# IlzeAmandaA/VAE-GP-ODE

Hardware: NVIDIA B200
Metric: GP-ODE RK4 latent traj-steps/s fwd+bwd (higher is better)
Workload: dtype f32

## Files before the change

### vae-gp-ode_b200/csrc/rbf_bwd_tc.cuh

```cuda
#pragma once

#include <cuda_bf16.h>
#include <cuda_fp16.h>

#include "rbf_kernels.cuh"
#include "tc_common.cuh"

namespace gpode {

#ifndef GPODE_BT_SLEEP_NS
#define GPODE_BT_SLEEP_NS 64
#endif
#ifndef GPODE_BT_A_TMEM
#define GPODE_BT_A_TMEM 1
#endif
constexpr int kBtACol = 448;
#ifndef GPODE_BT_EXP
#define GPODE_BT_EXP 0
#endif

constexpr int kBtStates = 128;
constexpr int kBtEpiWarps = 16;
constexpr int kBtEpi = kBtEpiWarps * 32;
constexpr int kBtFlushWarps = 4;
constexpr int kBtThreads = kBtEpi + 64 + 32 * kBtFlushWarps + 64;
constexpr int kBtPgIssuer = kBtEpiWarps + 2 + kBtFlushWarps;
constexpr int kBtThIssuer = kBtPgIssuer + 1;
constexpr int kBtTauBytes = 2 * 16 * 2048;
constexpr int kBtABytes = 3 * 4096;
constexpr int kBtXpBytes = 6 * 2048;
constexpr int kBtQCol = 256, kBtPgCol = 352;
constexpr int kBtNBars = 26;
constexpr uint32_t kBtOffTau = 0, kBtOffTh = 2 * kBtTauBytes, kBtOffP = kBtOffTh + 2 * kTcbThBytes, kBtOffA = kBtOffP + 2 * kTcbPBytes, kBtOffXp = kBtOffA + kBtABytes,
                   kBtOffXs = kBtOffXp + kBtXpBytes;

__host__ __device__ constexpr uint32_t tc_idesc_f16(int M, int N) {
  return (1u << 4) | (static_cast<uint32_t>(N >> 3) << 17) | (static_cast<uint32_t>(M >> 4) << 24);
}
__host__ __device__ constexpr uint32_t tc_idesc_bf16(int M, int N, int a_mn, int b_mn) {
  return (1u << 4) | (1u << 7) | (1u << 10) | (static_cast<uint32_t>(a_mn) << 15) | (static_cast<uint32_t>(b_mn) << 16) | (static_cast<uint32_t>(N >> 3) << 17) |
         (static_cast<uint32_t>(M >> 4) << 24);
}
__device__ __forceinline__ uint64_t tc_desc2(uint32_t saddr, uint32_t lbo_bytes, uint32_t sbo_bytes) {
  return static_cast<uint64_t>((saddr & 0x3FFFF) >> 4) | (static_cast<uint64_t>((lbo_bytes >> 4) & 0x3FFF) << 16) | (static_cast<uint64_t>((sbo_bytes >> 4) & 0x3FFF) << 32) |
         (static_cast<uint64_t>(1) << 46);
}
__device__ __forceinline__ void tcu_mma_f16(uint32_t d, uint64_t a, uint64_t b, uint32_t idesc, uint32_t acc) {
  asm volatile("{\n.reg .pred p, e;\nsetp.ne.b32 p, %4, 0;\nelect.sync _|e, 0xffffffff;\n@e tcgen05.mma.cta_group::1.kind::f16 [%0], %1, %2, %3, p;\n}\n" ::"r"(d), "l"(a), "l"(b),
               "r"(idesc), "r"(acc)
               : "memory");
}
__device__ __forceinline__ void tcu_mma_tf32(uint32_t d, uint64_t a, uint64_t b, uint32_t idesc, uint32_t acc) {
  asm volatile("{\n.reg .pred p, e;\nsetp.ne.b32 p, %4, 0;\nelect.sync _|e, 0xffffffff;\n@e tcgen05.mma.cta_group::1.kind::tf32 [%0], %1, %2, %3, p;\n}\n" ::"r"(d), "l"(a), "l"(b),
               "r"(idesc), "r"(acc)
               : "memory");
}
__device__ __forceinline__ void tcu_mma_f16_ts(uint32_t d, uint32_t a_tmem, uint64_t b, uint32_t idesc, uint32_t acc) {
  asm volatile("{\n.reg .pred p, e;\nsetp.ne.b32 p, %4, 0;\nelect.sync _|e, 0xffffffff;\n@e tcgen05.mma.cta_group::1.kind::f16 [%0], [%1], %2, %3, p;\n}\n" ::"r"(d), "r"(a_tmem),
               "l"(b), "r"(idesc), "r"(acc)
               : "memory");
}
__device__ __forceinline__ void tcu_mma_tf32_ts(uint32_t d, uint32_t a_tmem, uint64_t b, uint32_t idesc, uint32_t acc) {
  asm volatile("{\n.reg .pred p, e;\nsetp.ne.b32 p, %4, 0;\nelect.sync _|e, 0xffffffff;\n@e tcgen05.mma.cta_group::1.kind::tf32 [%0], [%1], %2, %3, p;\n}\n" ::"r"(d), "r"(a_tmem),
               "l"(b), "r"(idesc), "r"(acc)
               : "memory");
}
__device__ __forceinline__ void tc_st8(uint32_t taddr, const uint32_t (&r)[8]) {
  asm volatile("tcgen05.st.sync.aligned.32x32b.x8.b32 [%0], {%1,%2,%3,%4,%5,%6,%7,%8};" ::"r"(taddr), "r"(r[0]), "r"(r[1]), "r"(r[2]), "r"(r[3]), "r"(r[4]), "r"(r[5]),
               "r"(r[6]), "r"(r[7])
               : "memory");
}
__device__ __forceinline__ void tcu_commit(uint32_t bar) {
  asm volatile("{\n.reg .pred e;\nelect.sync _|e, 0xffffffff;\n@e tcgen05.commit.cta_group::1.mbarrier::arrive::one.shared::cluster.b64 [%0];\n}\n" ::"r"(bar) : "memory");
}
__device__ __forceinline__ void tc_ld4(uint32_t taddr, float (&v)[4]) {
  uint32_t r0, r1, r2, r3;
  asm volatile("tcgen05.ld.sync.aligned.32x32b.x4.b32 {%0,%1,%2,%3}, [%4];" : "=r"(r0), "=r"(r1), "=r"(r2), "=r"(r3) : "r"(taddr));
  asm volatile("tcgen05.wait::ld.sync.aligned;" : "+r"(r0), "+r"(r1), "+r"(r2), "+r"(r3)::"memory");
  v[0] = __uint_as_float(r0);
  v[1] = __uint_as_float(r1);
  v[2] = __uint_as_float(r2);
  v[3] = __uint_as_float(r3);
}
__device__ __forceinline__ void tc_ld2(uint32_t taddr, float (&v)[2]) {
  uint32_t r0, r1;
  asm volatile("tcgen05.ld.sync.aligned.32x32b.x2.b32 {%0,%1}, [%2];" : "=r"(r0), "=r"(r1) : "r"(taddr));
  asm volatile("tcgen05.wait::ld.sync.aligned;" : "+r"(r0), "+r"(r1)::"memory");
  v[0] = __uint_as_float(r0);
  v[1] = __uint_as_float(r1);
}
__device__ __forceinline__ void tc_ld4_async(uint32_t taddr, uint32_t& r0, uint32_t& r1, uint32_t& r2, uint32_t& r3) {
  asm volatile("tcgen05.ld.sync.aligned.32x32b.x4.b32 {%0,%1,%2,%3}, [%4];" : "=r"(r0), "=r"(r1), "=r"(r2), "=r"(r3) : "r"(taddr));
}
__device__ __forceinline__ void tc_ld2_async(uint32_t taddr, uint32_t& r0, uint32_t& r1) {
  asm volatile("tcgen05.ld.sync.aligned.32x32b.x2.b32 {%0,%1}, [%2];" : "=r"(r0), "=r"(r1) : "r"(taddr));
}
__device__ __forceinline__ void tc_ld_fence(uint32_t (&r)[10]) {
  asm volatile("" : "+r"(r[0]), "+r"(r[1]), "+r"(r[2]), "+r"(r[3]), "+r"(r[4]), "+r"(r[5]), "+r"(r[6]), "+r"(r[7]), "+r"(r[8]), "+r"(r[9])::"memory");
}
__device__ __forceinline__ void sts128(uint32_t saddr, uint32_t a, uint32_t b, uint32_t c, uint32_t d) {
#if GPODE_BT_EXP
  if (GPODE_BT_EXP & 8) {
    asm volatile("" ::"r"(saddr), "r"(a), "r"(b), "r"(c), "r"(d));
    return;
  }
#endif
  asm volatile("st.shared.v4.b32 [%0], {%1,%2,%3,%4};" ::"r"(saddr), "r"(a), "r"(b), "r"(c), "r"(d) : "memory");
}
__device__ __forceinline__ void bt_split2(float v0, float v1, uint32_t& hd, uint32_t& rm) {
  hd = __byte_perm(__float_as_uint(v0), __float_as_uint(v1), 0x7632);
  const float2 l = fma2(make_float2(__uint_as_float(__float_as_uint(v0) & 0xFFFF0000u), __uint_as_float(__float_as_uint(v1) & 0xFFFF0000u)), bc(-1.f), make_float2(v0, v1));
  asm("cvt.rn.bf16x2.f32 %0, %1, %2;" : "=r"(rm) : "f"(l.y), "f"(l.x));
}

#ifdef GPODE_BT_PROFILE
#define BT_E0 long long et_[12] = {0, 0, 0, 0, 0, 0, 0, 0, 0, 0, 0, 0}, ec_ = clock64();
#define BT_E(i) { const long long now_ = clock64(); et_[i] += now_ - ec_; ec_ = now_; }
#define BT_EPRINT if (blockIdx.x == 5 && blockIdx.y == 0 && b0 == static_cast<long>(n) && (tid == 0 || tid == 480)) \
  printf("bwd tc epilogue warp %d (cycles per item): first wait %lld, wait tau_empty %lld, ld issue + ld wait + arrives %lld, math+store %lld (+ wait next theta %lld), k setup + xprime %lld (+ wait xp_empty %lld), pg red %lld (+ waits pg_full / q_full %lld), q epilogue %lld (+ %lld)\n", warp, \
         et_[0] / n, et_[1] / n, et_[2] / n, et_[3] / n, et_[7] / n, et_[4] / n, et_[8] / n, et_[5] / n, et_[9] / n, et_[6] / n, et_[10] / n);
#define BT_I0 long long it_[8] = {0, 0, 0, 0, 0, 0, 0, 0}, ic_ = clock64();
#define BT_I(i) { const long long now_ = clock64(); it_[i] += now_ - ic_; ic_ = now_; }
#define BT_IPRINT if (blockIdx.x == 5 && blockIdx.y == 0 && b0 == static_cast<long>(n) && lane == 0) \
  printf("bwd tc issuer (cycles per item): theta waits (tile, acc_empty) %lld, theta issue %lld, wait tau_full %lld, wait p tile %lld, wait q_empty/xp/pg_empty %lld, issue Q %lld, issue PG %lld\n", \
         it_[0] / n, it_[1] / n, it_[2] / n, it_[3] / n, it_[4] / n, it_[5] / n, it_[6] / n);
#else
#define BT_E0
#define BT_E(i)
#define BT_EPRINT
#define BT_I0
#define BT_I(i)
#define BT_IPRINT
#endif

struct BwdTcSmem {
  unsigned char* tau;
  unsigned char* th;
  unsigned char* pp;
  unsigned char* A;
  unsigned char* xp;
  float* xs;
  float* dx;
  float* hdr;
  float* dell;
  float* dvar;
  float* sk;
  float* gs;
  float* g_pg;
  float* g_dnu;
  uint64_t* bars;
  uint32_t sb;
  uint32_t sbars;
  uint32_t* tmem_slot;
  const float* tiles;
  uint32_t tmem;
  long blk;
  long kk;
  long pgc;
  long total;
};

inline int rbf_bwd_tc_smem_bytes(const RbfGeom& g) {
  return 2 * kBtTauBytes + 2 * kTcbThBytes + 2 * kTcbPBytes + kBtABytes + kBtXpBytes + 2 * 16 * kBtStates * 4 + (g.D_out * g.hdr_floats + g.D_out * (g.DP + 1) + g.D_out + 8) * 4 +
         kBtNBars * 8 + 64 + 1024;
}

template <int DP_>
struct RbfTcBwdPolicy {
  static constexpr int DP = DP_;
  static constexpr int R = 1;
  static constexpr int kThreads = kBtThreads;
  static constexpr int kMinBlocks = 1;
  static constexpr int kStateThreads = kBtStates;
  static constexpr int kXsStride = kBtStates;
  static constexpr bool kCoopGlue = true;
  static constexpr int kThreadsBwd = kBtThreads;
  static constexpr int kMinBlocksBwd = 1;
  using Geom = RbfGeom;
  using Accum = RbfAccum;
  using Smem = BwdTcSmem;
  static_assert(DP_ <= 16, "one 16-wide K block per operand part");

  __device__ static __forceinline__ uint32_t th_full(const Smem& sm, int s) { return sm.sbars + 8u * static_cast<uint32_t>(s); }
  __device__ static __forceinline__ uint32_t th_empty(const Smem& sm, int s) { return sm.sbars + 8u * static_cast<uint32_t>(2 + s); }
  __device__ static __forceinline__ uint32_t p_full(const Smem& sm, int s) { return sm.sbars + 8u * static_cast<uint32_t>(4 + s); }
  __device__ static __forceinline__ uint32_t p_empty(const Smem& sm, int s) { return sm.sbars + 8u * static_cast<uint32_t>(6 + s); }
  __device__ static __forceinline__ uint32_t acc_full(const Smem& sm, int a) { return sm.sbars + 8u * static_cast<uint32_t>(8 + a); }
  __device__ static __forceinline__ uint32_t acc_empty(const Smem& sm, int a) { return sm.sbars + 8u * static_cast<uint32_t>(10 + a); }
  __device__ static __forceinline__ uint32_t tau_full(const Smem& sm, int a) { return sm.sbars + 8u * static_cast<uint32_t>(12 + a); }
  __device__ static __forceinline__ uint32_t tau_empty(const Smem& sm, int a) { return sm.sbars + 8u * static_cast<uint32_t>(14 + a); }
  __device__ static __forceinline__ uint32_t q_full(const Smem& sm, int q) { return sm.sbars + 8u * static_cast<uint32_t>(16 + q); }
  __device__ static __forceinline__ uint32_t q_empty(const Smem& sm, int q) { return sm.sbars + 8u * static_cast<uint32_t>(18 + q); }
  __device__ static __forceinline__ uint32_t pg_full(const Smem& sm, int q) { return sm.sbars + 8u * static_cast<uint32_t>(20 + q); }
  __device__ static __forceinline__ uint32_t pg_empty(const Smem& sm, int q) { return sm.sbars + 8u * static_cast<uint32_t>(22 + q); }
  __device__ static __forceinline__ uint32_t xp_full(const Smem& sm) { return sm.sbars + 8u * 24u; }
  __device__ static __forceinline__ uint32_t xp_empty(const Smem& sm) { return sm.sbars + 8u * 25u; }

  __device__ static __forceinline__ Smem carve(float* smem, const Geom& g) {
    Smem s;
    uint32_t pad = (1024u - (smem_u32(smem) & 1023u)) & 1023u;
    asm volatile("" : "+r"(pad));
    unsigned char* base = reinterpret_cast<unsigned char*>(smem) + pad;
    s.sb = smem_u32(base);
    asm volatile("" : "+r"(s.sb));
    s.tau = base;
    s.th = s.tau + 2 * kBtTauBytes;
    s.pp = s.th + 2 * kTcbThBytes;
    s.A = s.pp + 2 * kTcbPBytes;
    s.xp = s.A + kBtABytes;
    s.xs = reinterpret_cast<float*>(s.xp + kBtXpBytes);
    s.dx = reinterpret_cast<float*>(s.xp);
    s.hdr = s.xs + 16 * kBtStates;
    s.dell = s.hdr + g.D_out * g.hdr_floats;
    s.dvar = s.dell + g.D_out * DP;
    s.sk = s.dvar + g.D_out;
    s.gs = s.sk + ((g.D_out + 3) & ~3);
    float* end = s.gs + 16 * kBtStates;
    s.bars = reinterpret_cast<uint64_t*>(end + ((g.D_out * g.hdr_floats + g.D_out * (DP + 1)) & 1));
    s.sbars = smem_u32(s.bars);
    asm volatile("" : "+r"(s.sbars));
    s.tmem_slot = reinterpret_cast<uint32_t*>(s.bars + kBtNBars);
    s.g_pg = nullptr;
    s.g_dnu = nullptr;
    s.blk = 0;
    s.kk = 0;
    s.pgc = 0;
    return s;
  }

  __device__ static __forceinline__ void fetch_th(const Smem& sm, const Geom& g, long b) {
    const int per_eval = g.D_out * rbf_tcb_items(g);
    const int slot = static_cast<int>(b & 1);
    const float* src = sm.tiles + static_cast<size_t>(b % per_eval) * kTcbTileFloats;
    mbar_expect_tx(th_full(sm, slot), kTcbThBytes);
    bulk_g2s(sm.sb + kBtOffTh + slot * kTcbThBytes, src, kTcbThBytes, th_full(sm, slot));
  }
  __device__ static __forceinline__ void fetch_p(const Smem& sm, const Geom& g, long b) {
    const int per_eval = g.D_out * rbf_tcb_items(g);
    const int slot = static_cast<int>(b & 1);
    const float* src = sm.tiles + static_cast<size_t>(b % per_eval) * kTcbTileFloats + kTcbThFloats;
    mbar_expect_tx(p_full(sm, slot), kTcbPBytes);
    bulk_g2s(sm.sb + kBtOffP + slot * kTcbPBytes, src, kTcbPBytes, p_full(sm, slot));
  }

  __device__ static __forceinline__ long setup(Smem& sm, ChunkPipe&, const Geom& g, const float* packed, long n_evals, bool) {
    const int l = blockIdx.y, tid = threadIdx.x;
    const float* hdr = rbf_hdr_ptr(packed, g, l);
    for (int i = tid; i < g.D_out * g.hdr_floats; i += blockDim.x) sm.hdr[i] = hdr[i];
    for (int i = tid; i < 16 * kBtStates; i += blockDim.x) sm.xs[i] = 0.f;
    for (int i = tid; i < kBtXpBytes / 4; i += blockDim.x) reinterpret_cast<uint32_t*>(sm.xp)[i] = 0u;
    for (int i = tid; i < kBtABytes / 4; i += blockDim.x) reinterpret_cast<uint32_t*>(sm.A)[i] = 0u;
    for (int i = tid; i < g.D_out * (DP + 1); i += blockDim.x) sm.dell[i] = 0.f;
    for (int i = tid; i < g.D_out; i += blockDim.x) {
      float s, inv;
      rbf_pow2_scale(rbf_maxabs_ptr(packed, g, l)[i], s, inv);
      sm.sk[i] = inv;
    }
    sm.tiles = rbf_tcb_tiles_ptr(packed, g, l);
    sm.total = n_evals * g.D_out * rbf_tcb_items(g);
    if (tid == 0) {
      for (int i = 0; i < 2; ++i) {
        mbar_init(th_full(sm, i), 1);
        mbar_init(th_empty(sm, i), 1);
        mbar_init(p_full(sm, i), 1);
        mbar_init(p_empty(sm, i), 1);
        mbar_init(acc_full(sm, i), 1);
        mbar_init(acc_empty(sm, i), kBtEpiWarps);
        mbar_init(tau_full(sm, i), kBtEpiWarps);
        mbar_init(tau_empty(sm, i), 2);
        mbar_init(q_full(sm, i), 1);
        mbar_init(q_empty(sm, i), kBtFlushWarps);
        mbar_init(pg_full(sm, i), 1);
        mbar_init(pg_empty(sm, i), kBtFlushWarps);
      }
      mbar_init(xp_full(sm), kBtFlushWarps);
      mbar_init(xp_empty(sm), 1);
      mbar_fence_init();
    }
    if (tid < 32) {
      asm volatile("tcgen05.alloc.cta_group::1.sync.aligned.shared::cta.b32 [%0], %1;" ::"r"(smem_u32(sm.tmem_slot)), "r"(512) : "memory");
      asm volatile("tcgen05.relinquish_alloc_permit.cta_group::1.sync.aligned;" ::: "memory");
    }
    asm volatile("fence.proxy.async.shared::cta;" ::: "memory");
    asm volatile("tcgen05.fence::before_thread_sync;" ::: "memory");
    __syncthreads();
    asm volatile("tcgen05.fence::after_thread_sync;" ::: "memory");
    sm.tmem = *sm.tmem_slot;
    if (tid == kBtEpi + 32) {
      for (long f = 0; f < 2 && f < sm.total; ++f) {
        fetch_th(sm, g, f);
        fetch_p(sm, g, f);
      }
    }
    return sm.total;
  }

  __device__ static __forceinline__ void finish(Smem&) {}

  __device__ static __forceinline__ void flush(const Smem& sm, const Geom& g, const Accum& acc) {
    for (int i = threadIdx.x; i < g.D_out * DP; i += blockDim.x) atomicAdd(&acc.dell_x[i], sm.dell[i]);
    for (int i = threadIdx.x; i < g.D_out; i += blockDim.x) atomicAdd(&acc.dvar[i], sm.dvar[i]);
    asm volatile("tcgen05.fence::before_thread_sync;" ::: "memory");
    __syncthreads();
    if (threadIdx.x < 32) asm volatile("tcgen05.dealloc.cta_group::1.sync.aligned.b32 %0, %1;" ::"r"(sm.tmem), "r"(512) : "memory");
  }

  __device__ static __forceinline__ void bind(Smem& sm, const Accum& acc) {
    sm.g_pg = acc.pg;
    sm.g_dnu = acc.dnu;
  }

  __device__ static __forceinline__ void vjp(ChunkPipe&, const Geom& g, long, Smem& sm, const States<R>& st, const float* gvec, const float* fvec,
                                             const float* fpvec, long kstride, long sstride) {
    const int tid = threadIdx.x, lane = tid & 31;
    const int warp = __shfl_sync(0xffffffffu, tid >> 5, 0);
    const int nbs = rbf_tcb_items_s(g), nbi = rbf_tcb_items(g), nbm = nbi - nbs;
    const int n = g.D_out * nbi;
    const long b0 = sm.blk, kk0 = sm.kk, pg0 = sm.pgc;
    (void)st;
    if (tid < kBtStates) {
      float xv[16], mx = 0.f;
#pragma unroll
      for (int d = 0; d < 16; ++d) {
        xv[d] = d < DP ? sm.xs[d * kBtStates + tid] : 0.f;
        mx = fmaxf(mx, fabsf(xv[d]));
      }
      float sn, inv;
      rbf_pow2_scale(mx, sn, inv);
#if !GPODE_BT_A_TMEM
#pragma unroll
      for (int c = 0; c < 2; ++c) {
        uint32_t hh[4], ll[4];
#pragma unroll
        for (int i = 0; i < 4; ++i) {
          const float v0 = xv[8 * c + 2 * i] * sn, v1 = xv[8 * c + 2 * i + 1] * sn;
          const __half2 h = __floats2half2_rn(v0, v1);
          const __half2 lo_ = __floats2half2_rn(v0 - __low2float(h), v1 - __high2float(h));
          hh[i] = *reinterpret_cast<const uint32_t*>(&h);
          ll[i] = *reinterpret_cast<const uint32_t*>(&lo_);
        }
        sts128(sm.sb + kBtOffA + c * 2048 + tid * 16, hh[0], hh[1], hh[2], hh[3]);
        sts128(sm.sb + kBtOffA + 4096 + c * 2048 + tid * 16, ll[0], ll[1], ll[2], ll[3]);
      }
      sts128(sm.sb + kBtOffA + 8192 + tid * 16, __float_as_uint(sn), __float_as_uint(sn), 0u, 0u);
#endif
#if GPODE_BT_A_TMEM
      {
        uint32_t th_[8], tl_[8], ts_[8];
#pragma unroll
        for (int i = 0; i < 8; ++i) {
          const float v0 = xv[2 * i] * sn, v1 = xv[2 * i + 1] * sn;
          const __half2 h = __floats2half2_rn(v0, v1);
          const __half2 lo_ = __floats2half2_rn(v0 - __low2float(h), v1 - __high2float(h));
          th_[i] = *reinterpret_cast<const uint32_t*>(&h);
          tl_[i] = *reinterpret_cast<const uint32_t*>(&lo_);
          ts_[i] = i < 2 ? __float_as_uint(sn) : 0u;
        }
        const uint32_t ta_ = sm.tmem + kBtACol + (static_cast<uint32_t>((tid >> 5) * 32) << 16);
        tc_st8(ta_, th_);
        tc_st8(ta_ + 8, tl_);
        tc_st8(ta_ + 16, ts_);
        asm volatile("tcgen05.wait::st.sync.aligned;" ::: "memory");
        asm volatile("tcgen05.fence::before_thread_sync;" ::: "memory");
      }
#endif
    }
    if (tid < kBtEpi) {
#pragma unroll 4
      for (int e = tid; e < g.D_out * kBtStates; e += kBtEpi) {
        const int k = e / kBtStates, sl = e - k * kBtStates;
        const long n_st = static_cast<long>(blockIdx.x) * kBtStates + sl;
        const bool live_st = n_st < g.N;
        const long at = k * kstride + (static_cast<long>(blockIdx.y) * g.N + (live_st ? n_st : g.N - 1)) * sstride;
        const float gk = live_st ? gvec[at] : 0.f;
        sm.gs[e] = gk;
        const float v = warp_sum(gk * (fvec[at] - 0.5f * fpvec[at]));
        if (lane == 0) atomicAdd(&sm.dvar[k], v);
      }
    }
    asm volatile("fence.proxy.async.shared::cta;" ::: "memory");
    __syncthreads();
    const int q = warp >> 2;
    int sidx = 32 * (warp & 3) + lane;
    asm volatile("" : "+r"(sidx));
    if (warp == kBtEpiWarps + 1) {
      if (lane == 0) {
        const long end = min(sm.total, b0 + n + 2);
        for (long f = b0; f < end; ++f) {
          if (f + 2 < end) {
            tc_wait(th_empty(sm, static_cast<int>(f & 1)), static_cast<uint32_t>((f >> 1) & 1));
            fetch_th(sm, g, f + 2);
          }
          if (f >= b0 + 2) {
            tc_wait(p_empty(sm, static_cast<int>(f & 1)), static_cast<uint32_t>(((f - 2) >> 1) & 1));
            fetch_p(sm, g, f);
          }
        }
      }
    } else if (warp == kBtEpiWarps) {
      const uint32_t aTau = sm.sb + kBtOffTau, aP = sm.sb + kBtOffP;
      constexpr uint32_t id_q = tc_idesc_bf16(128, kTcbQN, 0, 0);
      BT_I0
      int k = 0, j = 0;
#pragma unroll 1
      for (int i = 0; i < n; ++i) {
        const long b = b0 + i;
        const int slot = static_cast<int>(b & 1);
        const long kk = kk0 + k;
        tc_wait(tau_full(sm, slot), static_cast<uint32_t>((b >> 1) & 1));
        BT_I(2)
        tc_wait(p_full(sm, slot), static_cast<uint32_t>((b >> 1) & 1));
        BT_I(3)
        if (j == 0 && kk >= 2) tc_wait(q_empty(sm, static_cast<int>(kk & 1)), static_cast<uint32_t>(((kk - 2) >> 1) & 1));
        BT_I(4)
        asm volatile("tcgen05.fence::after_thread_sync;" ::: "memory");
        const uint32_t ta = aTau + slot * kBtTauBytes, bp = aP + slot * kTcbPBytes;
        const uint32_t dq = sm.tmem + kBtQCol + static_cast<uint32_t>(kk & 1) * kTcbQN;
#pragma unroll
        for (int s = 0; s < ((GPODE_BT_EXP & 2) ? 0 : 16); ++s)
          tcu_mma_f16(dq, tc_desc2(ta + s * 2 * 2048, 2048, 128), tc_desc2(bp + (s & 7) * 2 * kTcbQN * 16, kTcbQN * 16, 128), id_q, (j > 0 || s > 0) ? 1u : 0u);
        tcu_commit(p_empty(sm, slot));
        if (j == nbi - 1) tcu_commit(q_full(sm, static_cast<int>(kk & 1)));
        BT_I(5)
        tcu_commit(tau_empty(sm, slot));
        BT_I(6)
        if (++j == nbi) {
          j = 0;
          ++k;
        }
      }
      BT_IPRINT
    } else if (warp == kBtThIssuer) {
      const uint32_t aA = sm.sb + kBtOffA, aTh = sm.sb + kBtOffTh;
      constexpr uint32_t id_th = tc_idesc_f16(128, kTcbUnits), id_off = tc_idesc(128, kTcbUnits);
      BT_I0
      auto issue_theta = [&](long b) {
        const int slot = static_cast<int>(b & 1);
        tc_wait(th_full(sm, slot), static_cast<uint32_t>((b >> 1) & 1));
        if (b >= 2) tc_wait(acc_empty(sm, slot), static_cast<uint32_t>(((b - 2) >> 1) & 1));
        BT_I(0)
        asm volatile("tcgen05.fence::after_thread_sync;" ::: "memory");
        const uint32_t d = sm.tmem + slot * kTcbUnits, bt = aTh + slot * kTcbThBytes;
        if (!(GPODE_BT_EXP & 16)) {
#if GPODE_BT_A_TMEM
        tcu_mma_f16_ts(d, sm.tmem + kBtACol, tc_desc2(bt, 2048, 128), id_th, 0u);
        tcu_mma_f16_ts(d, sm.tmem + kBtACol + 8, tc_desc2(bt, 2048, 128), id_th, 1u);
        tcu_mma_f16_ts(d, sm.tmem + kBtACol, tc_desc2(bt + 4096, 2048, 128), id_th, 1u);
        tcu_mma_tf32_ts(d, sm.tmem + kBtACol + 16, tc_desc2(bt + 8192, 2048, 128), id_off, 1u);
        (void)aA;
#else
        tcu_mma_f16(d, tc_desc2(aA, 2048, 128), tc_desc2(bt, 2048, 128), id_th, 0u);
        tcu_mma_f16(d, tc_desc2(aA + 4096, 2048, 128), tc_desc2(bt, 2048, 128), id_th, 1u);
        tcu_mma_f16(d, tc_desc2(aA, 2048, 128), tc_desc2(bt + 4096, 2048, 128), id_th, 1u);
        tcu_mma_tf32(d, tc_desc2(aA + 8192, 2048, 128), tc_desc2(bt + 8192, 2048, 128), id_off, 1u);
#endif
        }
        tcu_commit(acc_full(sm, slot));
        tcu_commit(th_empty(sm, slot));
        BT_I(1)
      };
#pragma unroll 1
      for (int i = 0; i < n; ++i) issue_theta(b0 + i);
    } else if (warp == kBtPgIssuer) {
      const uint32_t aTau = sm.sb + kBtOffTau, aXp = sm.sb + kBtOffXp;
      constexpr uint32_t id_pg = tc_idesc_bf16(128, kTcbQN, 1, 1);
      int k = 0, j = 0;
#pragma unroll 1
      for (int i = 0; i < n; ++i) {
        const long b = b0 + i;
        const int slot = static_cast<int>(b & 1);
        const long kk = kk0 + k;
        tc_wait(tau_full(sm, slot), static_cast<uint32_t>((b >> 1) & 1));
        if (j >= nbs) {
          const long pc = pg0 + static_cast<long>(k) * nbm + (j - nbs);
          if (j == nbs) tc_wait(xp_full(sm), static_cast<uint32_t>(kk & 1));
          if (pc >= 2) tc_wait(pg_empty(sm, static_cast<int>(pc & 1)), static_cast<uint32_t>(((pc - 2) >> 1) & 1));
          asm volatile("tcgen05.fence::after_thread_sync;" ::: "memory");
          const uint32_t ta = aTau + slot * kBtTauBytes;
          const uint32_t dpg = sm.tmem + kBtPgCol + static_cast<uint32_t>(pc & 1) * kTcbQN;
#pragma unroll
          for (int p = 0; p < ((GPODE_BT_EXP & 1) ? 0 : 2); ++p)
#pragma unroll
            for (int s = 0; s < 8; ++s)
              tcu_mma_f16(dpg, tc_desc2(ta + p * 16 * 2048 + s * 2 * 128, 128, 2048), tc_desc2(aXp + s * 2 * 128, 128, 2048), id_pg, (p > 0 || s > 0) ? 1u : 0u);
          tcu_commit(pg_full(sm, static_cast<int>(pc & 1)));
          if (j == nbi - 1) tcu_commit(xp_empty(sm));
        }
        tcu_commit(tau_empty(sm, slot));
        if (++j == nbi) {
          j = 0;
          ++k;
        }
      }
    } else if (warp >= kBtEpiWarps + 2 && warp < kBtPgIssuer) {
      const uint32_t lane_base = static_cast<uint32_t>((warp & 3) * 32) << 16;
      const uint32_t aXp = sm.sb + kBtOffXp;
      const uint32_t tq0 = sm.tmem + kBtQCol + lane_base, tp0 = sm.tmem + kBtPgCol + lane_base;
      float dxa[16];
#pragma unroll
      for (int d = 0; d < 16; ++d) dxa[d] = 0.f;
      auto write_xprime = [&](int k, long kk) {
        if (kk >= 1) mbar_wait_sleepy(xp_empty(sm), static_cast<uint32_t>((kk - 1) & 1), GPODE_BT_SLEEP_NS);
        const float gk = sm.gs[k * kBtStates + sidx];
        const uint32_t row = aXp + sidx * 16;
#pragma unroll
        for (int c = 0; c < 2; ++c) {
          uint32_t hd[4], rm[4];
#pragma unroll
          for (int v = 0; v < 4; ++v) {
            const int d = 8 * c + 2 * v;
            bt_split2(d < DP ? gk * sm.xs[d * kBtStates + sidx] : 0.f, d + 1 < DP ? gk * sm.xs[(d + 1) * kBtStates + sidx] : 0.f, hd[v], rm[v]);
          }
          sts128(row + c * 2048, hd[0], hd[1], hd[2], hd[3]);
          sts128(row + (2 + c) * 2048, rm[0], rm[1], rm[2], rm[3]);
        }
        uint32_t hg, lg;
        bt_split2(gk, 0.f, hg, lg);
        asm volatile("st.shared.b32 [%0], %1;" ::"r"(row + 4 * 2048), "r"((hg & 0xFFFFu) | (lg << 16)) : "memory");
        asm volatile("fence.proxy.async.shared::cta;" ::: "memory");
        __syncwarp();
        if (lane == 0) tc_arrive(xp_full(sm));
      };
      write_xprime(0, kk0);
      long pc = pg0;
#pragma unroll 1
      for (int k = 0; k < g.D_out; ++k) {
        const long kk = kk0 + k;
#pragma unroll 1
        for (int jm = 0; jm < nbm; ++jm, ++pc) {
          mbar_wait_sleepy(pg_full(sm, static_cast<int>(pc & 1)), static_cast<uint32_t>((pc >> 1) & 1), GPODE_BT_SLEEP_NS);
          asm volatile("tcgen05.fence::after_thread_sync;" ::: "memory");
          const uint32_t tp = tp0 + static_cast<uint32_t>(pc & 1) * kTcbQN;
          uint32_t ph[16], pl[16], ps0, ps1;
          tc_ld16_async(tp, ph);
          tc_ld16_async(tp + 16, pl);
          tc_ld2_async(tp + 32, ps0, ps1);
          asm volatile("tcgen05.wait::ld.sync.aligned;" ::: "memory");
          asm volatile("" : "+r"(ps0), "+r"(ps1)::"memory");
          tc_ld_wait(ph);
          tc_ld_wait(pl);
          asm volatile("tcgen05.fence::before_thread_sync;" ::: "memory");
          __syncwarp();
          if (lane == 0) tc_arrive(pg_empty(sm, static_cast<int>(pc & 1)));
          const int unit = jm * kTcbUnits + sidx;
          if (unit < g.M) {
            const size_t base = (static_cast<size_t>(blockIdx.y) * g.D_out + k) * (2 * g.MP2) + unit;
            float* dst = sm.g_pg + base * DP;
            if constexpr (DP == 16) {
#pragma unroll
              for (int c = 0; c < 4; ++c)
                asm volatile("red.global.add.v4.f32 [%0], {%1,%2,%3,%4};" ::"l"(dst + 4 * c), "f"(__uint_as_float(ph[4 * c]) + __uint_as_float(pl[4 * c])),
                             "f"(__uint_as_float(ph[4 * c + 1]) + __uint_as_float(pl[4 * c + 1])), "f"(__uint_as_float(ph[4 * c + 2]) + __uint_as_float(pl[4 * c + 2])),
                             "f"(__uint_as_float(ph[4 * c + 3]) + __uint_as_float(pl[4 * c + 3]))
                             : "memory");
            } else {
#pragma unroll
              for (int d = 0; d < DP; ++d) asm volatile("red.global.add.f32 [%0], %1;" ::"l"(dst + d), "f"(__uint_as_float(ph[d]) + __uint_as_float(pl[d])) : "memory");
            }
            asm volatile("red.global.add.f32 [%0], %1;" ::"l"(sm.g_dnu + base), "f"(__uint_as_float(ps0) + __uint_as_float(ps1)) : "memory");
          }
        }
        if (k + 1 < g.D_out) write_xprime(k + 1, kk + 1);
        const float gk = sm.gs[k * kBtStates + sidx];
        mbar_wait_sleepy(q_full(sm, static_cast<int>(kk & 1)), static_cast<uint32_t>((kk >> 1) & 1), GPODE_BT_SLEEP_NS);
        asm volatile("tcgen05.fence::after_thread_sync;" ::: "memory");
        {
          const uint32_t tq = tq0 + static_cast<uint32_t>(kk & 1) * kTcbQN;
          uint32_t qh[16], ql[16], qs0, qs1;
          tc_ld16_async(tq, qh);
          tc_ld16_async(tq + 16, ql);
          tc_ld2_async(tq + 32, qs0, qs1);
          asm volatile("tcgen05.wait::ld.sync.aligned;" ::: "memory");
          asm volatile("" : "+r"(qs0), "+r"(qs1)::"memory");
          tc_ld_wait(qh);
          tc_ld_wait(ql);
          asm volatile("tcgen05.fence::before_thread_sync;" ::: "memory");
          __syncwarp();
          if (lane == 0) tc_arrive(q_empty(sm, static_cast<int>(kk & 1)));
          const float es = __uint_as_float(qs0) + __uint_as_float(qs1);
          const float* hdr_k = sm.hdr + k * g.hdr_floats;
          float red[16];
#pragma unroll
          for (int d = 0; d < 16; ++d) {
            red[d] = 0.f;
            if (d < DP) {
              const float xd = sm.xs[d * kBtStates + sidx];
              const float dxk = gk * fmaf(2.f * hdr_k[d] * xd, es, __uint_as_float(qh[d]) + __uint_as_float(ql[d]));
              dxa[d] += dxk;
              red[d] = xd * dxk;
            }
          }
#pragma unroll
          for (int o = 16; o > 0; o >>= 1)
#pragma unroll
            for (int d = 0; d < DP; ++d) red[d] += __shfl_xor_sync(0xffffffffu, red[d], o);
          float rv = 0.f;
#pragma unroll
          for (int d = 0; d < DP; ++d) rv = lane == d ? red[d] : rv;
          if (lane < DP) atomicAdd(&sm.dell[k * DP + lane], rv);
        }
      }
      sm.blk = b0 + n;
      sm.kk = kk0 + g.D_out;
      sm.pgc = pg0 + static_cast<long>(g.D_out) * nbm;
      __syncthreads();
#pragma unroll
      for (int d = 0; d < DP; ++d) sm.dx[d * kBtStates + sidx] = dxa[d];
      __syncthreads();
      return;
    } else {
      const uint32_t lane_base = static_cast<uint32_t>((warp & 3) * 32) << 16;
      float mx = 0.f;
#pragma unroll
      for (int d = 0; d < DP; ++d) mx = fmaxf(mx, fabsf(sm.xs[d * kBtStates + sidx]));
      float sn_, inv_n;
      rbf_pow2_scale(mx, sn_, inv_n);
      float Ak = 0.f, inv_s = 1.f;
      const uint32_t aTau = sm.sb + kBtOffTau;
      const uint32_t ta0 = sm.tmem + q * 32 + lane_base;
      int k = 0, j = 0;
      uint32_t rA[16], rB[16];
      const uint32_t b0u = static_cast<uint32_t>(b0);
      int i_wait = b0 >= 2 ? 0 : static_cast<int>(2 - b0);
      asm volatile("" : "+r"(i_wait));
      tc_wait(acc_full(sm, static_cast<int>(b0u & 1)), (b0u >> 1) & 1u);
      asm volatile("tcgen05.fence::after_thread_sync;" ::: "memory");
      tc_ld16_async(ta0 + (b0u & 1) * kTcbUnits, rA);
      uint32_t b = b0u;
#pragma unroll 1
      for (int i = 0; i < n; ++i, ++b) {
        const int slot = static_cast<int>(b & 1);
        const bool is_k = j >= nbs;
        if (j == 0) {
          const float* hdr_k = sm.hdr + k * g.hdr_floats;
          Ak = 0.f;
#pragma unroll
          for (int d = 0; d < DP; ++d) {
            const float xv = sm.xs[d * kBtStates + sidx];
            Ak = fmaf(hdr_k[d] * xv, xv, Ak);
          }
          inv_s = inv_n * sm.sk[k];
        }
        if (i >= i_wait) tc_wait(tau_empty(sm, slot), ((b - 2u) >> 1) & 1u);
        tc_ld_wait(rA);
        asm volatile("tcgen05.fence::after_thread_sync;" ::: "memory");
        tc_ld16_async(ta0 + slot * kTcbUnits + 16, rB);
        const float addk = is_k ? Ak : 0.f;
        const uint32_t trow = aTau + slot * kBtTauBytes + sidx * 16 + (4 * q) * 2048;
#pragma unroll
        for (int c = 0; c < 2; ++c) {
          uint32_t hd[4], rm[4];
#pragma unroll
          for (int v = 0; v < 4; ++v) {
            const float2 tt = fma2(make_float2(__uint_as_float(rA[8 * c + 2 * v]), __uint_as_float(rA[8 * c + 2 * v + 1])), bc(inv_s), bc(addk));
            const float t0 = tt.x, t1 = tt.y;
            bt_split2((GPODE_BT_EXP & 4) ? t0 : (is_k ? ex2_approx(t0) : __cosf(t0)), (GPODE_BT_EXP & 4) ? t1 : (is_k ? ex2_approx(t1) : __cosf(t1)), hd[v], rm[v]);
          }
          sts128(trow + c * 2048, hd[0], hd[1], hd[2], hd[3]);
          sts128(trow + (16 + c) * 2048, rm[0], rm[1], rm[2], rm[3]);
        }
        tc_ld_wait(rB);
        asm volatile("tcgen05.fence::before_thread_sync;" ::: "memory");
        __syncwarp();
        if (lane == 0) tc_arrive(acc_empty(sm, slot));
        if (i + 1 < n) {
          tc_wait(acc_full(sm, slot ^ 1), ((b + 1u) >> 1) & 1u);
          asm volatile("tcgen05.fence::after_thread_sync;" ::: "memory");
          tc_ld16_async(ta0 + (slot ^ 1) * kTcbUnits, rA);
        }
#pragma unroll
        for (int c = 0; c < 2; ++c) {
          uint32_t hd[4], rm[4];
#pragma unroll
          for (int v = 0; v < 4; ++v) {
            const float2 tt = fma2(make_float2(__uint_as_float(rB[8 * c + 2 * v]), __uint_as_float(rB[8 * c + 2 * v + 1])), bc(inv_s), bc(addk));
            const float t0 = tt.x, t1 = tt.y;
            bt_split2((GPODE_BT_EXP & 4) ? t0 : (is_k ? ex2_approx(t0) : __cosf(t0)), (GPODE_BT_EXP & 4) ? t1 : (is_k ? ex2_approx(t1) : __cosf(t1)), hd[v], rm[v]);
          }
          sts128(trow + (2 + c) * 2048, hd[0], hd[1], hd[2], hd[3]);
          sts128(trow + (18 + c) * 2048, rm[0], rm[1], rm[2], rm[3]);
        }
        if (!(GPODE_BT_EXP & 32)) asm volatile("fence.proxy.async.shared::cta;" ::: "memory");
        __syncwarp();
        if (lane == 0) tc_arrive(tau_full(sm, slot));
        if (++j == nbi) {
          j = 0;
          ++k;
        }
      }
    }
    sm.blk = b0 + n;
    sm.kk = kk0 + g.D_out;
    sm.pgc = pg0 + static_cast<long>(g.D_out) * nbm;
    __syncthreads();
    __syncthreads();
  }
};

}
```

Measured before the change: 21.60 million.

## Keep tau operand in tensor memory for Q MMA, write smem only for PG

The epilogue now writes the transformed tau values back into the same TMEM accumulator columns with tcgen05.st instead of only to shared memory. The Q MMA reads its A operand from TMEM through a ts-form MMA with a column map, and shared-memory stores happen only for the kernel items the PG MMA needs. Barrier counts change so that acc_empty is signalled by the MMA commit instead of the epilogue warps. The aim is to cut shared-memory store traffic and proxy fences on the cosine items. In exchange the epilogue must wait for tcgen05 stores to complete, and slot reuse now depends on the MMA finishing reading TMEM.

```diff
diff --git a/vae-gp-ode_b200/csrc/rbf_bwd_tc.cuh b/vae-gp-ode_b200/csrc/rbf_bwd_tc.cuh
--- a/vae-gp-ode_b200/csrc/rbf_bwd_tc.cuh
+++ b/vae-gp-ode_b200/csrc/rbf_bwd_tc.cuh
@@ -15,6 +15,15 @@
 #define GPODE_BT_A_TMEM 1
 #endif
 constexpr int kBtACol = 448;
+#ifndef GPODE_BT_LATE_PF
+#define GPODE_BT_LATE_PF 0
+#endif
+#ifndef GPODE_BT_PG_AFTER_TH
+#define GPODE_BT_PG_AFTER_TH 0
+#endif
+#ifndef GPODE_BT_PG_AFTER_Q
+#define GPODE_BT_PG_AFTER_Q 0
+#endif
 #ifndef GPODE_BT_EXP
 #define GPODE_BT_EXP 0
 #endif
@@ -30,6 +39,13 @@
 constexpr int kBtABytes = 3 * 4096;
 constexpr int kBtXpBytes = 6 * 2048;
 constexpr int kBtQCol = 256, kBtPgCol = 352;
+constexpr int kBtTmemCols = 512;
+static_assert(kBtQCol == 2 * kTcbUnits, "the two theta / tau slots come first");
+static_assert(kBtPgCol == kBtQCol + 2 * kTcbQN && kBtACol == kBtPgCol + 2 * kTcbQN, "Q, PG and the theta state operand follow without overlap");
+static_assert(kBtACol + 24 <= kBtTmemCols, "tensor-memory plan exceeds the allocation");
+static_assert(kTcbUnits == 4 * 32 && kBtEpiWarps == 16, "tau in place: epilogue warp w owns slot columns 32 (w >> 2) .. + 31 of lane quarter w & 3");
+__host__ __device__ constexpr uint32_t bt_tau_col(int s) { return 32u * ((s & 7) >> 1) + 16u * (s & 1) + 8u * (s >> 3); }
+static_assert(bt_tau_col(0) == 0 && bt_tau_col(8) == 8 && bt_tau_col(1) == 16 && bt_tau_col(9) == 24 && bt_tau_col(15) == 120, "tau column map");
 constexpr int kBtNBars = 26;
 constexpr uint32_t kBtOffTau = 0, kBtOffTh = 2 * kBtTauBytes, kBtOffP = kBtOffTh + 2 * kTcbThBytes, kBtOffA = kBtOffP + 2 * kTcbPBytes, kBtOffXp = kBtOffA + kBtABytes,
                    kBtOffXs = kBtOffXp + kBtXpBytes;
@@ -265,9 +281,9 @@
         mbar_init(p_full(sm, i), 1);
         mbar_init(p_empty(sm, i), 1);
         mbar_init(acc_full(sm, i), 1);
-        mbar_init(acc_empty(sm, i), kBtEpiWarps);
+        mbar_init(acc_empty(sm, i), 1);
         mbar_init(tau_full(sm, i), kBtEpiWarps);
-        mbar_init(tau_empty(sm, i), 2);
+        mbar_init(tau_empty(sm, i), 1);
         mbar_init(q_full(sm, i), 1);
         mbar_init(q_empty(sm, i), kBtFlushWarps);
         mbar_init(pg_full(sm, i), 1);
@@ -278,7 +294,7 @@
       mbar_fence_init();
     }
     if (tid < 32) {
-      asm volatile("tcgen05.alloc.cta_group::1.sync.aligned.shared::cta.b32 [%0], %1;" ::"r"(smem_u32(sm.tmem_slot)), "r"(512) : "memory");
+      asm volatile("tcgen05.alloc.cta_group::1.sync.aligned.shared::cta.b32 [%0], %1;" ::"r"(smem_u32(sm.tmem_slot)), "r"(kBtTmemCols) : "memory");
       asm volatile("tcgen05.relinquish_alloc_permit.cta_group::1.sync.aligned;" ::: "memory");
     }
     asm volatile("fence.proxy.async.shared::cta;" ::: "memory");
@@ -302,7 +318,7 @@
     for (int i = threadIdx.x; i < g.D_out; i += blockDim.x) atomicAdd(&acc.dvar[i], sm.dvar[i]);
     asm volatile("tcgen05.fence::before_thread_sync;" ::: "memory");
     __syncthreads();
-    if (threadIdx.x < 32) asm volatile("tcgen05.dealloc.cta_group::1.sync.aligned.b32 %0, %1;" ::"r"(sm.tmem), "r"(512) : "memory");
+    if (threadIdx.x < 32) asm volatile("tcgen05.dealloc.cta_group::1.sync.aligned.b32 %0, %1;" ::"r"(sm.tmem), "r"(kBtTmemCols) : "memory");
   }
 
   __device__ static __forceinline__ void bind(Smem& sm, const Accum& acc) {
@@ -398,7 +414,7 @@
         }
       }
     } else if (warp == kBtEpiWarps) {
-      const uint32_t aTau = sm.sb + kBtOffTau, aP = sm.sb + kBtOffP;
+      const uint32_t aP = sm.sb + kBtOffP;
       constexpr uint32_t id_q = tc_idesc_bf16(128, kTcbQN, 0, 0);
       BT_I0
       int k = 0, j = 0;
@@ -414,15 +430,15 @@
         if (j == 0 && kk >= 2) tc_wait(q_empty(sm, static_cast<int>(kk & 1)), static_cast<uint32_t>(((kk - 2) >> 1) & 1));
         BT_I(4)
         asm volatile("tcgen05.fence::after_thread_sync;" ::: "memory");
-        const uint32_t ta = aTau + slot * kBtTauBytes, bp = aP + slot * kTcbPBytes;
+        const uint32_t ta = sm.tmem + slot * kTcbUnits, bp = aP + slot * kTcbPBytes;
         const uint32_t dq = sm.tmem + kBtQCol + static_cast<uint32_t>(kk & 1) * kTcbQN;
 #pragma unroll
         for (int s = 0; s < ((GPODE_BT_EXP & 2) ? 0 : 16); ++s)
-          tcu_mma_f16(dq, tc_desc2(ta + s * 2 * 2048, 2048, 128), tc_desc2(bp + (s & 7) * 2 * kTcbQN * 16, kTcbQN * 16, 128), id_q, (j > 0 || s > 0) ? 1u : 0u);
+          tcu_mma_f16_ts(dq, ta + bt_tau_col(s), tc_desc2(bp + (s & 7) * 2 * kTcbQN * 16, kTcbQN * 16, 128), id_q, (j > 0 || s > 0) ? 1u : 0u);
         tcu_commit(p_empty(sm, slot));
         if (j == nbi - 1) tcu_commit(q_full(sm, static_cast<int>(kk & 1)));
         BT_I(5)
-        tcu_commit(tau_empty(sm, slot));
+        tcu_commit(acc_empty(sm, slot));
         BT_I(6)
         if (++j == nbi) {
           j = 0;
@@ -471,6 +487,12 @@
         const int slot = static_cast<int>(b & 1);
         const long kk = kk0 + k;
         tc_wait(tau_full(sm, slot), static_cast<uint32_t>((b >> 1) & 1));
+#if GPODE_BT_PG_AFTER_Q
+        if (j >= nbs) tc_wait(acc_empty(sm, slot), static_cast<uint32_t>((b >> 1) & 1));
+#endif
+#if GPODE_BT_PG_AFTER_TH
+        if (j >= nbs && i + 2 < n) tc_wait(acc_full(sm, slot), static_cast<uint32_t>(((b + 2) >> 1) & 1));
+#endif
         if (j >= nbs) {
           const long pc = pg0 + static_cast<long>(k) * nbm + (j - nbs);
           if (j == nbs) tc_wait(xp_full(sm), static_cast<uint32_t>(kk & 1));
@@ -646,43 +668,57 @@
         asm volatile("tcgen05.fence::after_thread_sync;" ::: "memory");
         tc_ld16_async(ta0 + slot * kTcbUnits + 16, rB);
         const float addk = is_k ? Ak : 0.f;
+        const bool to_smem = is_k;
         const uint32_t trow = aTau + slot * kBtTauBytes + sidx * 16 + (4 * q) * 2048;
+        uint32_t tv[16];
 #pragma unroll
         for (int c = 0; c < 2; ++c) {
-          uint32_t hd[4], rm[4];
 #pragma unroll
           for (int v = 0; v < 4; ++v) {
             const float2 tt = fma2(make_float2(__uint_as_float(rA[8 * c + 2 * v]), __uint_as_float(rA[8 * c + 2 * v + 1])), bc(inv_s), bc(addk));
             const float t0 = tt.x, t1 = tt.y;
-            bt_split2((GPODE_BT_EXP & 4) ? t0 : (is_k ? ex2_approx(t0) : __cosf(t0)), (GPODE_BT_EXP & 4) ? t1 : (is_k ? ex2_approx(t1) : __cosf(t1)), hd[v], rm[v]);
-          }
-          sts128(trow + c * 2048, hd[0], hd[1], hd[2], hd[3]);
-          sts128(trow + (16 + c) * 2048, rm[0], rm[1], rm[2], rm[3]);
-        }
+            bt_split2((GPODE_BT_EXP & 4) ? t0 : (is_k ? ex2_approx(t0) : __cosf(t0)), (GPODE_BT_EXP & 4) ? t1 : (is_k ? ex2_approx(t1) : __cosf(t1)), tv[4 * c + v], tv[8 + 4 * c + v]);
+          }
+          if (to_smem) {
+            sts128(trow + c * 2048, tv[4 * c], tv[4 * c + 1], tv[4 * c + 2], tv[4 * c + 3]);
+            sts128(trow + (16 + c) * 2048, tv[8 + 4 * c], tv[8 + 4 * c + 1], tv[8 + 4 * c + 2], tv[8 + 4 * c + 3]);
+          }
+        }
+        tc_st16(ta0 + slot * kTcbUnits, tv);
         tc_ld_wait(rB);
-        asm volatile("tcgen05.fence::before_thread_sync;" ::: "memory");
-        __syncwarp();
-        if (lane == 0) tc_arrive(acc_empty(sm, slot));
+#if !GPODE_BT_LATE_PF
         if (i + 1 < n) {
           tc_wait(acc_full(sm, slot ^ 1), ((b + 1u) >> 1) & 1u);
           asm volatile("tcgen05.fence::after_thread_sync;" ::: "memory");
           tc_ld16_async(ta0 + (slot ^ 1) * kTcbUnits, rA);
         }
+#endif
 #pragma unroll
         for (int c = 0; c < 2; ++c) {
-          uint32_t hd[4], rm[4];
 #pragma unroll
           for (int v = 0; v < 4; ++v) {
             const float2 tt = fma2(make_float2(__uint_as_float(rB[8 * c + 2 * v]), __uint_as_float(rB[8 * c + 2 * v + 1])), bc(inv_s), bc(addk));
             const float t0 = tt.x, t1 = tt.y;
-            bt_split2((GPODE_BT_EXP & 4) ? t0 : (is_k ? ex2_approx(t0) : __cosf(t0)), (GPODE_BT_EXP & 4) ? t1 : (is_k ? ex2_approx(t1) : __cosf(t1)), hd[v], rm[v]);
-          }
-          sts128(trow + (2 + c) * 2048, hd[0], hd[1], hd[2], hd[3]);
-          sts128(trow + (18 + c) * 2048, rm[0], rm[1], rm[2], rm[3]);
-        }
-        if (!(GPODE_BT_EXP & 32)) asm volatile("fence.proxy.async.shared::cta;" ::: "memory");
+            bt_split2((GPODE_BT_EXP & 4) ? t0 : (is_k ? ex2_approx(t0) : __cosf(t0)), (GPODE_BT_EXP & 4) ? t1 : (is_k ? ex2_approx(t1) : __cosf(t1)), tv[4 * c + v], tv[8 + 4 * c + v]);
+          }
+          if (to_smem) {
+            sts128(trow + (2 + c) * 2048, tv[4 * c], tv[4 * c + 1], tv[4 * c + 2], tv[4 * c + 3]);
+            sts128(trow + (18 + c) * 2048, tv[8 + 4 * c], tv[8 + 4 * c + 1], tv[8 + 4 * c + 2], tv[8 + 4 * c + 3]);
+          }
+        }
+        tc_st16(ta0 + slot * kTcbUnits + 16, tv);
+        asm volatile("tcgen05.wait::st.sync.aligned;" ::: "memory");
+        asm volatile("tcgen05.fence::before_thread_sync;" ::: "memory");
+        if (to_smem && !(GPODE_BT_EXP & 32)) asm volatile("fence.proxy.async.shared::cta;" ::: "memory");
         __syncwarp();
         if (lane == 0) tc_arrive(tau_full(sm, slot));
+#if GPODE_BT_LATE_PF
+        if (i + 1 < n) {
+          tc_wait(acc_full(sm, slot ^ 1), ((b + 1u) >> 1) & 1u);
+          asm volatile("tcgen05.fence::after_thread_sync;" ::: "memory");
+          tc_ld16_async(ta0 + (slot ^ 1) * kTcbUnits, rA);
+        }
+#endif
         if (++j == nbi) {
           j = 0;
           ++k;
```

Measured after the change: 18.76 million, median of 6. 13.1% lower.
